# davidesantangelo/krep

Measured on AMD Instinct MI355X. Metric: GB/s scanned (literal scan, match offsets produced), haystack resident in HBM, higher is better.
Workload: dtype u8; 1 GPU; literal8: 8-byte case-sensitive literal 'Sherlock', ~1e-4 matches/byte, offsets tracked; 32 GiB per GPU (BASELINE.json configs[1]); pattern=Sherlock, bytes_per_gpu=34359738368, matches=3436005, parallelism=contiguous shards x1, start-offset ownership, 1 RCCL all-reduce of counts

## Files before the change

### include/krep_gpu_debug.h

```cpp
#ifndef KREP_GPU_DEBUG_H
#define KREP_GPU_DEBUG_H
#include "krep_gpu.h"
#ifdef __cplusplus
extern "C" {
#endif

uint64_t krep_gpu_debug_replay_host(int krep_ref_algo, const void *text, size_t n, const void *pattern, uint32_t m,
                                    int whole_word, size_t cur, int open_line);
void krep_gpu_debug_force_rounds(int rounds);
void krep_gpu_debug_force_stage_cap(int records);
void krep_gpu_debug_force_single_grid(int blocks);
uint64_t krep_gpu_debug_single_failovers(void);
uint64_t krep_gpu_debug_single_launches(void);
uint64_t krep_gpu_debug_tiny_launches(void);
uint64_t krep_gpu_debug_tiny_dense_launches(void);
void krep_gpu_debug_inject_failure(int kind);
void krep_gpu_debug_chain_fixups(uint64_t *rescans, uint64_t *replays);
void krep_gpu_debug_fold_carry(const krep_gpu_seq_carry_t *in, const krep_gpu_seq_carry_t *piece, krep_gpu_seq_carry_t *out);
uint64_t krep_gpu_debug_anchored_launches(void);
uint64_t krep_gpu_debug_literal_dma_launches(void);
int krep_gpu_debug_literal_dma_state(const krep_gpu_plan_t *plan, int *looked, int *barred, double *pass_rate);
uint64_t krep_gpu_debug_runs_launches(void);
int krep_gpu_debug_split_state(const krep_gpu_plan_t *plan);
int krep_gpu_debug_anchor_info(const krep_gpu_plan_t *plan, int *state, uint32_t *moved, double *rate_end_grams, double *rate_anchors);
int krep_gpu_debug_anchor_measured(const krep_gpu_plan_t *plan, double *measured, int *resamples);

#ifdef __cplusplus
}
#endif
#endif
```

### krep_amd/csrc/kg_config.hip

```cpp
#include <hip/hip_runtime.h>

#include <algorithm>
#include <atomic>
#include <chrono>
#include <cstdarg>
#include <cstdio>
#include <cstdlib>
#include <cstring>
#include <mutex>
#include <string>
#include <vector>

#include "../../include/krep_gpu.h"
#include "kg_common.h"
#include "kg_internal.h"
#include "kg_plan.h"
#include "kg_replay.h"

using namespace kg;

static thread_local std::string g_err;
namespace kg {
int fail(const char *fmt, ...)
{
// ... 204 lines not shown
namespace kg {
extern int g_s1_force_grid;
std::atomic<uint64_t> g_fused1_failovers{0};
}
extern "C" void krep_gpu_debug_force_single_grid(int blocks) { kg::g_s1_force_grid = blocks < 0 ? 0 : blocks; }
extern "C" uint64_t krep_gpu_debug_single_failovers(void) { return g_fused1_failovers.load(); }
namespace kg {
std::atomic<uint64_t> g_fused1_launches{0};
}
extern "C" uint64_t krep_gpu_debug_single_launches(void) { return kg::g_fused1_launches.load(); }
namespace kg {
std::atomic<uint64_t> g_tiny_launches{0};
}
extern "C" uint64_t krep_gpu_debug_tiny_launches(void) { return kg::g_tiny_launches.load(); }
namespace kg {
std::atomic<uint64_t> g_tiny_dense_launches{0};
}
extern "C" uint64_t krep_gpu_debug_tiny_dense_launches(void) { return kg::g_tiny_dense_launches.load(); }
namespace kg {
std::atomic<uint64_t> g_ac_anchored_launches{0};
}
extern "C" uint64_t krep_gpu_debug_anchored_launches(void) { return kg::g_ac_anchored_launches.load(); }
extern "C" uint64_t krep_gpu_debug_literal_dma_launches(void) { return kg::g_lit_dma_launches.load(); }
extern "C" uint64_t krep_gpu_debug_runs_launches(void) { return kg::g_runs_launches.load(); }
```

### krep_amd/csrc/kg_internal.h

```cpp
#pragma once
#include <hip/hip_runtime.h>

#include <atomic>
#include <cstring>
#include <initializer_list>
#include <mutex>
#include <vector>

#include "../../include/krep_gpu.h"
#include "../../include/krep_gpu_debug.h"
#include "kg_common.h"

namespace kg {

int fail(const char *fmt, ...);
const char *device_unusable(int device);
bool inject(int kind);
#define HIPCHK(x)                                                                                 \
    do                                                                                            \
    {                                                                                             \
        hipError_t e_ = (x);                                                                      \
        if (e_ != hipSuccess)                                                                     \
            return kg::fail("%s failed: %s (%s:%d)", #x, hipGetErrorString(e_), __FILE__, __LINE__); \
    } while (0)
// ... 24 lines not shown

template <auto Kernel> hipError_t grant_dynamic_lds(int bytes)
{
    static std::atomic<bool> granted[64];
    int dev = 0;
    (void)hipGetDevice(&dev);
    const bool known = dev >= 0 && dev < 64;
    if (known && granted[dev].load(std::memory_order_acquire))
        return hipSuccess;
    const hipError_t e = hipFuncSetAttribute(reinterpret_cast<const void *>(Kernel), hipFuncAttributeMaxDynamicSharedMemorySize, bytes);
    if (e == hipSuccess && known)
        granted[dev].store(true, std::memory_order_release);
    return e;
}

hipError_t launch_literal(const LitArgs &a, uint32_t num_cu, hipStream_t st);
int runs_count_greedy(const uint8_t *d_text, uint64_t text_len, uint64_t lo, uint64_t hi, uint32_t m, uint8_t byte, bool ci, int num_cu,
                      unsigned long long *d_slots, unsigned long long *h_slots, hipStream_t st, uint64_t *total, uint64_t *end_p1);
bool literal_dma_eligible(const LitArgs &a);
hipError_t launch_literal_dma(const LitArgs &a, uint32_t num_cu, hipStream_t st);
hipError_t launch_dma_byte_look(const uint8_t *text, uint64_t lo, uint32_t n_cells, uint32_t prefilter, bool ci, unsigned long long *out, hipStream_t st);
extern std::atomic<uint64_t> g_runs_launches;
extern std::atomic<uint64_t> g_lit_dma_launches;

struct PostScratch;
constexpr int kFusedShapeMax = 5;
double single_fused_max_density(int shape);
int single_fused_shape_for(double density, double margin, int start);
bool single_fused_reopens(uint64_t total, uint64_t span);
constexpr int kFusedGaveUp = 1;
int single_fused_run(const LitArgs &a, uint64_t n_units, uint64_t span, PostScratch &post, Counters *d_ctr, Counters *h_ctr,
                     uint32_t num_cu, int *shape, hipEvent_t ev_end, hipStream_t st, bool count_launch);

struct PostScratch
{
    unsigned long long *d_unitinfo = nullptr;
    unsigned long long *d_offsets = nullptr;
    unsigned long long *d_blk = nullptr;
    uint64_t units_cap = 0;
    unsigned long long *d_stage = nullptr;
    uint64_t stage_cap_words = 0;
    uint64_t *d_occ = nullptr;
    uint64_t occ_cap = 0;
    uint8_t *d_keep = nullptr;
    unsigned long long *d_gblk = nullptr;
    unsigned long long *d_surv = nullptr;
// ... 119 lines not shown
```

### krep_amd/csrc/kg_literal_dma.hip

```cpp
#include <hip/hip_runtime.h>
#include <algorithm>
#include <atomic>
#include <cstdlib>
#include "kg_common.h"
#include "kg_device.h"
#include "kg_internal.h"

namespace kg {

namespace {

constexpr u32 kDmaPark = 80;
constexpr u32 kDmaRing = 2u * kSegBytes;
constexpr u32 kDmaTail = 256u;
constexpr u32 kDmaWaveLds = kDmaRing + kDmaTail;
}

template <int KIND, bool MASKED, bool CI>
__global__ __launch_bounds__(kBlock, 2) void lit_scan_dma(const LitArgs a)
{
    extern __shared__ __attribute__((aligned(16))) uint8_t d_smem[];
    __shared__ u64 s_info_all[kWavesPerBlk][kDmaPark];
    __shared__ __attribute__((aligned(16))) unsigned short s_slots_all[kWavesPerBlk][kDmaPark * 16u];
    __shared__ u32 s_unit_all[kWavesPerBlk][kDmaPark];
    const u32 lane = lane_id();
    const u32 wave = __builtin_amdgcn_readfirstlane(threadIdx.x >> 6);
    uint8_t *ring = d_smem + wave * kDmaWaveLds;
    uint8_t *tailb = ring + kDmaRing;
    u64 *s_info = s_info_all[wave];
    unsigned short *s_slots = s_slots_all[wave];
    u32 *s_unit = s_unit_all[wave];
    const u32 ring_lds = (u32)(size_t)(__attribute__((address_space(3))) uint8_t *)ring;

    const bool want_pos = (a.flags & F_POS) != 0;
    const bool ww = (a.flags & F_WW) != 0;
    const u64 hi_match = (a.own_hi < a.text_len - a.m + 1) ? a.own_hi : (a.text_len - a.m + 1);
    constexpr u64 kUnitBytes = (u64)kRoundsBig * kSegBytes;
    const u64 n_units = a.num_tiles * kWavesPerBlk;

    const bool park = want_pos && a.stage_cap >= 16u && a.stage_cap <= 128u && (a.stage_cap & 7u) == 0u && n_units < (1ull << 32);
    const u32 park_max = park ? kDmaPark * 16u / a.stage_cap : 0u;
    u32 n_park = 0;
    auto flush_parked = [&]() __attribute__((always_inline)) {
        for (u32 i = lane; i < n_park; i += 64u)
        {
            const u64 u = s_unit[i];
            a.unitinfo[u] = s_info[i];
            if (s_info[i] & kUiCountMask)
            {
// ... 17 lines not shown
        const u64 u = static_next;
        static_next += (u64)gridDim.x * kWavesPerBlk;
        return u;
    };
    auto issue_round = [&](u64 seg, u32 buf) -> bool {
        if (seg + kSegBytes > a.text_len)
            return false;
        const uint8_t *src = a.text + seg + lane * 16u;
        uint8_t *dst = ring + buf * kSegBytes;
#pragma unroll
        for (int j = 0; j < kCells; ++j)
            __builtin_amdgcn_global_load_lds((const __attribute__((address_space(1))) void *)(src + j * kCellBytes),
                                             (__attribute__((address_space(3))) void *)(dst + j * kCellBytes), 16, 0, 2 );
        return true;
    };
    auto issue_tail = [&](u64 at) -> bool {
        if (at + kDmaTail > a.text_len)
            return false;
        __builtin_amdgcn_global_load_lds((const __attribute__((address_space(1))) void *)(a.text + at + lane * 4u),
                                         (__attribute__((address_space(3))) void *)tailb, 4, 0, 0);
        return true;
    };

    u64 acc_total = 0;
    u32 pf_cells = 0;
    u32 wcnt = 0;
    auto stage_hit = [&](u64 unit, u32 idx, u32 rel) __attribute__((always_inline)) {
        if (idx < a.stage_cap)
        {
            unsigned short *slot = park ? &s_slots[n_park * a.stage_cap] : reinterpret_cast<unsigned short *>(a.stage) + unit * (u64)a.stage_cap;
            slot[idx] = (unsigned short)rel;
        }
    };
    auto publish = [&](u64 unit) __attribute__((always_inline)) {
        acc_total += wcnt;
        if (want_pos)
        {
            if (lane == 0)
            {
                const u64 info = (u64)wcnt | (wcnt ? (kLnHead | kLnTail) : 0ull);
                if (park)
                {
                    s_info[n_park] = info;
                    s_unit[n_park] = (u32)unit;
                }
                else
                    a.unitinfo[unit] = info;
                if (wcnt > a.stage_cap)
                {
                    atomicAdd(&a.ctr->overflow_units, 1ull);
                    atomicMax(&a.ctr->max_unit_count, (u64)wcnt);
                }
            }
            if (park && ++n_park == park_max)
                flush_parked();
        }
        wcnt = 0;
    };
    auto exact = [&](u32 A0, u32 A4) -> bool {
        const u32 e0 = CI ? (A0 | a.l0) : A0;
        bool h = (KIND == 4 && MASKED) ? (((e0 ^ a.p0) & a.k0) == 0u) : (e0 == a.p0);
        if (KIND >= 8)
        {
            const u32 e4 = CI ? (A4 | a.l1) : A4;
            h = h && ((KIND == 8 && MASKED) ? (((e4 ^ a.p1) & a.k1) == 0u) : (e4 == a.p1));
        }
        return h;
    };
    auto owned = [&](u64 p) -> bool { return p >= a.own_lo && p < hi_match && !(p >= a.excl_lo && p < a.excl_hi); };
    auto word_ok = [&](u64 p) -> bool {
        if (p > 0 && p != a.ww_exempt_left && is_wordc(a.text[p - 1]))
            return false;
        if (p + a.m < a.text_len && is_wordc(a.text[p + a.m]))
            return false;
        return true;
    };
    auto boundary = [&](u64 seg_prev, u64 unit, u32 r_prev, u32 c0, u32 c1, u32 n0, u32 n1) __attribute__((always_inline)) {
        {
            const u32 f = 0x01010101u * ((CI ? (a.p0 | 0x20u) : a.p0) & 0xffu);
            const u32 y0 = (CI ? (c0 | 0x20202020u) : c0) ^ f, y1 = (CI ? (c1 | 0x20202020u) : c1) ^ f;
// ... 75 lines not shown
                             : "+v"(x[0]), "+v"(x[1]), "+v"(x[2]), "+v"(x[3]), "+v"(x[4]), "+v"(x[5]), "+v"(x[6]), "+v"(x[7]), "+v"(y[0]), "+v"(y[1]),
                               "+v"(y[2]), "+v"(y[3]), "+v"(y[4]), "+v"(y[5]), "+v"(y[6]), "+v"(y[7])
                             :
                             : "memory");
#pragma unroll
                for (int j = 0; j < kCells; ++j)
                {
                    vv[j] = make_uint4(x[j].x, x[j].y, x[j].z, x[j].w);
                    nn[j] = make_uint2(y[j].x, y[j].y);
                }
            }
            else
            {
#pragma unroll
                for (int j = 0; j < kCells; ++j)
                {
                    const W6 w = load_window_guarded(a.text, a.text_len, seg + (u64)j * kCellBytes + (u64)lane * 16u);
                    vv[j] = make_uint4(w.v[0], w.v[1], w.v[2], w.v[3]);
                    nn[j] = make_uint2(w.v[4], w.v[5]);
                }
            }
            if (deferred)
            {
                boundary(seg - kSegBytes, u0 + ((g - 1u) >> 2), (g - 1u) & 3u, c0, c1, __builtin_amdgcn_readfirstlane(vv[0].x),
                         __builtin_amdgcn_readfirstlane(vv[0].y));
                deferred = false;
                if (r == 0u)
                    publish(unit - 1u);
            }
            __builtin_amdgcn_sched_barrier(0);
#pragma unroll
            for (int j = 0; j < kCells; ++j)
            {
                const u64 lbase = seg + (u64)j * kCellBytes + (u64)lane * 16u;
                const u32 D[6] = {vv[j].x, vv[j].y, vv[j].z, vv[j].w, nn[j].x, nn[j].y};
                auto A = [&](int k) -> u32 {
                    return ((k & 3) == 0) ? D[k >> 2] : __builtin_amdgcn_alignbyte(D[(k >> 2) + 1], D[k >> 2], (u32)(k & 3));
                };
                u32 Dq[6];
#pragma unroll
                for (int w = 0; w < 6; ++w)
                    Dq[w] = CI ? (D[w] | 0x20202020u) : D[w];
                auto Aq = [&](int k) -> u32 {
                    return ((k & 3) == 0) ? Dq[k >> 2] : __builtin_amdgcn_alignbyte(Dq[(k >> 2) + 1], Dq[k >> 2], (u32)(k & 3));
                };
                const u32 p0q = CI ? (a.p0 | 0x20202020u) : a.p0;
                if (a.prefilter)
// ... 60 lines not shown
                            m16 &= ~(1u << k);
                    }
                }
                if (!__ballot(m16 != 0u))
                    continue;
                const u32 cnt = __popc(m16);
                u32 idx = wcnt, tot = 0;
                auto plane = [&](int b) {
                    const u64 bm = __ballot((cnt >> b) & 1u);
                    idx += mbcnt64(bm) << b;
                    tot += (u32)__popcll(bm) << b;
                };
                plane(0);
                plane(1);
                if (__ballot(cnt > 3u))
                {
                    plane(2);
                    plane(3);
                    plane(4);
                }
                wcnt += tot;
                if (want_pos)
                {
                    const u32 rel0 = (r * (u32)kCells + (u32)j) * kCellBytes + lane * 16u;
                    u32 rest = m16;
                    while (rest)
                    {
                        const u32 k = __builtin_ctz(rest);
                        rest &= rest - 1u;
                        stage_hit(unit, idx++, rel0 + k);
                    }
                }
            }
            if (dma_cur)
            {
                c0 = __builtin_amdgcn_readlane(vv[kCells - 1].z, 63);
                c1 = __builtin_amdgcn_readlane(vv[kCells - 1].w, 63);
                deferred = true;
            }
            if (g + 1u == nr)
            {
                if (deferred)
                {
                    u32 n0 = 0, n1 = 0;
                    if (tail_ok)
                    {
                        typedef u32 v2 __attribute__((ext_vector_type(2)));
                        v2 t;
                        const u32 taddr = ring_lds + kDmaRing;
                        asm volatile("ds_read_b64 %0, %1\n\ts_waitcnt lgkmcnt(0)" : "=v"(t) : "v"(taddr) : "memory");
                        n0 = __builtin_amdgcn_readfirstlane(t.x);
                        n1 = __builtin_amdgcn_readfirstlane(t.y);
                    }
                    else
                    {
                        const W6 w = load_window_guarded(a.text, a.text_len, seg + kSegBytes);
                        n0 = __builtin_amdgcn_readfirstlane(w.v[0]);
                        n1 = __builtin_amdgcn_readfirstlane(w.v[1]);
                    }
                    boundary(seg, unit, r, c0, c1, n0, n1);
                    deferred = false;
                }
                publish(unit);
            }
            else if (!deferred && r == 3u)
                publish(unit);
            dma_cur = dma_nx;
        }
        u0 = u_next;
    }
    if (park && n_park)
        flush_parked();
    if (lane == 0 && acc_total)
        atomicAdd(&a.ctr->total, acc_total);
    if (lane == 0 && pf_cells)
        atomicAdd(&a.ctr->candidates, (u64)pf_cells);
}

__global__ __launch_bounds__(256) void dma_byte_look(const uint8_t *text, u64 lo, u32 n_cells, u32 b4, u32 fold, unsigned long long *out)
{
    const u32 lane = lane_id();
    const u32 wave = blockIdx.x * 4u + (threadIdx.x >> 6), n_waves = gridDim.x * 4u;
    u32 cnt = 0;
    for (u32 c = wave; c < n_cells; c += n_waves)
    {
        const uint4 v = *reinterpret_cast<const uint4 *>(text + lo + (u64)c * kCellBytes + lane * 16u);
        const u32 d[4] = {v.x, v.y, v.z, v.w};
        u32 z = 0;
#pragma unroll
        for (int w = 0; w < 4; ++w)
        {
            const u32 y = (d[w] | fold) ^ b4;
            z |= (y - 0x01010101u) & ~y;
        }
        if (__ballot((z & 0x80808080u) != 0u))
            ++cnt;
    }
    if (lane == 0 && cnt)
        atomicAdd(out, (u64)cnt);
}
hipError_t launch_dma_byte_look(const uint8_t *text, uint64_t lo, uint32_t n_cells, uint32_t prefilter, bool ci, unsigned long long *out, hipStream_t st)
{
    hipLaunchKernelGGL(dma_byte_look, dim3(256), dim3(256), 0, st, text, (u64)lo, n_cells, prefilter, ci ? 0x20202020u : 0u, out);
    return hipGetLastError();
}

std::atomic<uint64_t> g_lit_dma_launches{0};

template <int KIND, bool MASKED, bool CI>
static hipError_t dma_launch3(const LitArgs &a, u32 num_cu, hipStream_t st)
{
    constexpr u32 lds = kWavesPerBlk * kDmaWaveLds;
    if (const hipError_t e = grant_dynamic_lds<&lit_scan_dma<KIND, MASKED, CI>>((int)lds); e != hipSuccess)
        return e;
    static const u32 bpc = [] { const char *e = getenv("KREP_GPU_LIT_DMA_BLOCKS_PER_CU"); return e && atoi(e) > 0 ? (u32)atoi(e) : 2u; }();
    const u32 grid = (u32)std::min<u64>(a.num_tiles, (u64)num_cu * bpc);
    hipLaunchKernelGGL((lit_scan_dma<KIND, MASKED, CI>), dim3(grid ? grid : 1), dim3(kBlock), lds, st, a);
    g_lit_dma_launches.fetch_add(1, std::memory_order_relaxed);
    return hipGetLastError();
}
template <int KIND, bool MASKED>
static hipError_t dma_launch2(const LitArgs &a, u32 num_cu, hipStream_t st)
{
    return (a.flags & F_CI) ? dma_launch3<KIND, MASKED, true>(a, num_cu, st) : dma_launch3<KIND, MASKED, false>(a, num_cu, st);
}

bool literal_dma_eligible(const LitArgs &a)
{
    return !getenv("KREP_GPU_LIT_NO_DMA") && a.prefilter != 0u && a.m >= 2 && a.m <= 8 && a.rounds == (u32)kRoundsBig && !(a.flags & F_LINES) && !a.emit_mode &&
           (a.upt >= 4 || getenv("KREP_GPU_LIT_DMA_ALL")) && a.text_len >= 4u * kSegBytes;
}
hipError_t launch_literal_dma(const LitArgs &a, u32 num_cu, hipStream_t st)
{
    if (a.m < 4)
        return dma_launch2<4, true>(a, num_cu, st);
    if (a.m == 4)
        return dma_launch2<4, false>(a, num_cu, st);
    if (a.m < 8)
        return dma_launch2<8, true>(a, num_cu, st);
    return dma_launch2<8, false>(a, num_cu, st);
}

}
```

### krep_amd/csrc/kg_plan.h

```cpp
#pragma once
#include <hip/hip_runtime.h>

#include <vector>

#include "../../include/krep_gpu.h"
#include "kg_common.h"
#include "kg_internal.h"

struct krep_gpu_plan
{
    krep_gpu_config_t cfg{};
    int device = 0;
    int ref_algo = KREP_RA_NONE;
    const char *unsupported = nullptr;
    bool only_matching = false;
    bool cs = true, ww = false, lines = false, track = false;
    size_t max_count = SIZE_MAX;
    std::vector<std::vector<uint8_t>> pats;
    uint32_t m = 0, p0 = 0, p1 = 0, k0 = 0, k1 = 0, l0 = 0, l1 = 0;
    uint32_t p2 = 0, p3 = 0, k2 = 0, k3 = 0, l2 = 0, l3 = 0;
    std::vector<uint8_t> pat_folded;
    bool has_border = false;
    bool has_newline = false;
    uint8_t *d_pat = nullptr;
    unsigned long long *d_pat_chunks = nullptr;
    uint32_t n_chunks = 0;
    kg::Counters *d_ctr = nullptr, *h_ctr = nullptr;
    int num_cu = 256;
    hipEvent_t ev0 = nullptr, ev1 = nullptr;
    kg::AcTables *ac = nullptr;
    kg::AcTables *ac_long = nullptr, *ac_short = nullptr;
    int ac_split = 0;
    match_position_t *d_split_rec = nullptr;
    uint64_t split_cap = 0;
    bool ac_has_newline = false;
    kg::PostScratch post;
    uint32_t sparse_cap = 16;
    bool dma_look_done = false;
    bool dma_off = false;
    const void *dma_off_text = nullptr;
    size_t dma_off_len = 0;
    double dma_pass_rate = 0;
    bool first_look_done = false;
    bool fused1_ok = true;
    bool fusedk_on = false;
    bool fusedk_never = false;
    int fusedk_shape = 0;
    int fused1_shape = 0;
    match_position_t *d_nl_rec = nullptr;
    uint64_t *d_nl_ln = nullptr;
    uint64_t nl_cap = 0;
    bool lines_list_off = false;
    kg::PostScratch aux;
    search_params_t sp{};
    std::vector<const char *> pat_ptrs;
    std::vector<size_t> pat_lens;
};
namespace kg {
struct Window
{
    const uint8_t *d_text;
    size_t text_len;
    size_t own_lo, own_hi;
    size_t global_base;
    size_t global_len;
// ... 7 lines not shown
```

### krep_amd/csrc/kg_scan.hip

```cpp
#include <hip/hip_runtime.h>

#include <algorithm>
#include <cstdio>
#include <cstdlib>
#include <cstring>
#include <vector>

#include "../../include/krep_gpu.h"
#include "kg_common.h"
#include "kg_internal.h"
#include "kg_plan.h"
#include "kg_replay.h"

using namespace kg;

struct Verdict { uint64_t ret, store; };
static Verdict verdict_for(int algo, const krep_gpu_plan *pl, uint64_t total, uint64_t lines, bool have_result)
{
    const size_t maxc = pl->max_count;
    const bool store = pl->track && have_result;
    Verdict v{0, 0};
    switch (algo)
    {
    case KREP_RA_MEMCHR:
// ... 213 lines not shown
          ps.excl_lo == ps.excl_hi && L.span() >= (1ull << 30) && !getenv("KREP_GPU_NO_FIRST_LOOK")))
        return 0;
    pl->first_look_done = true;
    const uint64_t span = L.span(), win = 2ull << 20, tile_bytes = (uint64_t)kRoundsBig * kSegBytes * kWavesPerBlk;
    HIPCHK(hipMemsetAsync(pl->d_ctr, 0, sizeof(Counters), st));
    uint64_t looked = 0;
    for (int q = 0; q < 2; ++q)
    {
        LitArgs sm = a;
        sm.flags &= ~(uint32_t)(F_POS | F_LINES);
        sm.stage_cap = 0;
        sm.upt = 0;
        sm.emit_mode = 0;
        sm.own_lo = (a.anchor + span / 4 * (2 * q + 1)) & ~(uint64_t)15;
        sm.own_hi = std::min<uint64_t>(L.hi_match, sm.own_lo + win);
        sm.anchor = sm.own_lo;
        sm.num_tiles = (sm.own_hi - sm.anchor + tile_bytes - 1) / tile_bytes;
        looked += sm.own_hi - sm.own_lo;
        HIPCHK(launch_literal(sm, (uint32_t)pl->num_cu, st));
    }
    HIPCHK(hipMemcpyAsync(pl->h_ctr, pl->d_ctr, sizeof(Counters), hipMemcpyDeviceToHost, st));
    HIPCHK(hipStreamSynchronize(st));
    const double density = looked ? (double)pl->h_ctr->total / (double)looked : 0.0, per_unit = density * 32768.0;
    if (m_scan == 1)
    {
        if (density > single_fused_max_density(kFusedShapeMax))
            pl->fused1_ok = false;
        else
            pl->fused1_shape = single_fused_shape_for(density, 1.05, 0);
    }
    else if (m_scan <= 8 && !pl->fusedk_never && per_unit >= fusedk_min_hits_per_unit() &&
             density <= single_fused_max_density(kFusedShapeMax))
    {
        pl->fusedk_on = true;
        pl->fusedk_shape = single_fused_shape_for(density, 1.05, 0);
    }
    else if (per_unit > 6.0)
        pl->sparse_cap = std::max<uint32_t>(pl->sparse_cap, per_unit > 100.0 ? 256u : per_unit > 40.0 ? 128u : 64u);
    if (getenv("KREP_GPU_DEBUG"))
        fprintf(stderr, "krep-gpu: first look: %.2f hits per 32-KiB unit in %llu sampled bytes -> one-pass %d (shape %d / %d), staging slot %u\n", per_unit,
                (unsigned long long)looked, (int)(m_scan == 1 ? pl->fused1_ok : pl->fusedk_on), pl->fused1_shape, pl->fusedk_shape, pl->sparse_cap);
    if ((a.flags & F_POS) && !L.fsc)
        a.stage_cap = a.rounds == kRoundsBig ? (m_scan == 1 ? 512u : pl->sparse_cap) : a.stage_cap;
    return 0;
}

// ... 15 lines not shown
    if (rc == 2)
        return 2;
    if (rc != kFusedGaveUp)
    {
        res->total = pl->h_ctr->total;
        res->summary = res->total ? (kLnHead | kLnTail) : 0;
        if (m_scan != 1 && L.density(res->total) * 32768.0 < 0.5 * fusedk_min_hits_per_unit())
            pl->fusedk_on = false;
        *done = true;
        return 0;
    }
    if (m_scan == 1)
        pl->fused1_ok = false;
    else
        pl->fusedk_on = false, pl->fusedk_never = true;
    g_fused1_failovers.fetch_add(1);
    return 0;
}

static void lit_learn_density(krep_gpu_plan *pl, const LitPass &ps, const LitScan &L)
{
    const LitArgs &a = L.a;
    const uint32_t m_scan = a.m;
    if ((a.flags & F_POS) && m_scan != 1 && a.rounds == kRoundsBig && pl->h_ctr->overflow_units * 64 > L.n_units && !L.fsc)
    {
        uint32_t want = 64;
        if (pl->sparse_cap >= 64)
            for (want = 128; want < 256 && want < pl->h_ctr->max_unit_count; want *= 2) {}
        pl->sparse_cap = std::max(pl->sparse_cap, want);
    }
    if ((a.flags & F_POS) && m_scan >= 2 && m_scan <= 8 && a.rounds == kRoundsBig && !L.fsc && !pl->fusedk_never &&
        ps.sink == LitPass::RECORDS && !ps.lines && L.hi_match > a.anchor)
    {
        const double density = L.density(pl->h_ctr->total);
        if (density * 32768.0 >= fusedk_min_hits_per_unit() && density <= single_fused_max_density(kFusedShapeMax))
        {
            pl->fusedk_on = true;
            pl->fusedk_shape = single_fused_shape_for(density, 1.0, 0);
        }
    }
    if (getenv("KREP_GPU_DEBUG") && (a.flags & F_POS))
        fprintf(stderr, "krep-gpu: literal scan: %llu of %llu units overflowed a %u-entry slot (fullest: %llu); one-pass next: %d (shape %d)\n",
                pl->h_ctr->overflow_units, (unsigned long long)L.n_units, a.stage_cap, pl->h_ctr->max_unit_count, (int)pl->fusedk_on,
                pl->fusedk_shape);
}
static void lit_reopen(krep_gpu_plan *pl, const LitScan &L)
{
    const uint32_t m_scan = L.a.m;
    if (!pl->fused1_ok && m_scan == 1 && single_fused_reopens(pl->h_ctr->total, L.span()))
        pl->fused1_ok = true;
    if (pl->fusedk_never && m_scan >= 2 && m_scan <= 8 && single_fused_reopens(pl->h_ctr->total, L.span()))
        pl->fusedk_never = false;
}

static int lit_two_pass(krep_gpu_plan *pl, const Window &w, const LitPass &ps, LitScan &L, bool chain, hipStream_t st)
{
    LitArgs &a = L.a;
    a.positions = ps.d_out;
    a.pos_cap = ps.sink == LitPass::RECORDS ? ps.out_cap : 0;
    HIPCHK(launch_literal(a, (uint32_t)pl->num_cu, st));
    if (chain && post_order(*ps.post, L.n_units, a.stage_cap, a.m, a.anchor + w.global_base, L.unit_bytes(), ps.lines, ps.d_out, a.pos_cap,
                            pl->d_ctr, pl->num_cu, st))
        return 2;
    if (ps.ev_end) HIPCHK(hipEventRecord(ps.ev_end, st));
    HIPCHK(hipMemcpyAsync(pl->h_ctr, pl->d_ctr, sizeof(Counters), hipMemcpyDeviceToHost, st));
    HIPCHK(hipStreamSynchronize(st));
    lit_dma_rate(pl, w, L);
    lit_learn_density(pl, ps, L);
    if ((a.flags & F_POS) && pl->h_ctr->overflow_units)
    {
        LitArgs e = a;
        e.emit_mode = 1;
        HIPCHK(hipMemsetAsync(&pl->d_ctr->ticket, 0, sizeof(unsigned long long), st));
        HIPCHK(launch_literal(e, (uint32_t)pl->num_cu, st));
        if (ps.ev_end) HIPCHK(hipEventRecord(ps.ev_end, st));
// ... 26 lines not shown
        }
    }
    return 0;
}

static int lit_pass(krep_gpu_plan *pl, const Window &w, const LitPass &ps, hipStream_t st, LitResult *res)
{
    *res = LitResult{};
    const uint32_t m_scan = ps.first_byte ? 1u : pl->m;
    size_t own_hi = std::min(ps.own_hi, w.text_len);
    if (ps.first_byte)
        own_hi = std::min<size_t>(own_hi, w.text_len - pl->m + 1);
    const uint64_t hi_match = std::min<uint64_t>(own_hi, w.text_len - m_scan + 1);
    if (hi_match <= ps.own_lo)
        return 0;
    LitScan L = lit_args(pl, w, ps, own_hi, hi_match);
    if (lit_dma_look(pl, w, ps, L, st))
        return 2;
    res->n_units = L.n_units;
    res->unit_bytes = L.unit_bytes();
    res->anchor = L.a.anchor;
    bool done = false;
    if (lit_first_look(pl, ps, L, st) || lit_one_pass(pl, w, ps, L, st, res, &done))
        return 2;
    if (done)
        return 0;
    const bool chain = (L.a.flags & (F_POS | F_LINES)) != 0;
    if (chain)
    {
        PostScratch &post = *ps.post;
        if (post_reserve(post, L.n_units, (L.n_units * L.a.stage_cap + 3) / 4))
            return 2;
        L.a.unitinfo = post.d_unitinfo;
        L.a.stage = (uint64_t *)post.d_stage;
        L.a.offsets = (const uint64_t *)post.d_offsets;
    }
    HIPCHK(hipMemsetAsync(pl->d_ctr, 0, sizeof(Counters), st));
    if (ps.sink != LitPass::OCC ? lit_two_pass(pl, w, ps, L, chain, st) : lit_two_pass_occ(pl, w, ps, L, st))
        return 2;
    res->total = pl->h_ctr->total;
    res->lines = pl->h_ctr->lines;
    lit_reopen(pl, L);
    res->summary = chain ? pl->h_ctr->summary : (res->total ? (kLnHead | kLnTail) : 0);
    return 0;
}

// ... 774 lines not shown
```

### krep_amd/csrc/kg_tickets.h

```cpp
#pragma once
#include <hip/hip_runtime.h>
#include "kg_common.h"
#include "kg_device.h"

namespace kg {

constexpr unsigned long long kTkReady = 1ull << 63;
constexpr uint32_t kTkSpinLimit = 1u << 24;
constexpr uint32_t kTkResolveChunk = 8;

__device__ __forceinline__ void tk_resolve(unsigned long long *__restrict__ agg, unsigned long long *__restrict__ pref,
                                           const unsigned long long n_tickets, Counters *ctr, const uint32_t lane)
{
    u64 running = 0, base = 0;
    u32 spins = 0;
    while (base < n_tickets)
    {
        const u64 mine = base + (u64)lane * kTkResolveChunk;
        u64 v[kTkResolveChunk];
        u32 lead = 0, nvalid = 0;
        bool run = true;
#pragma unroll
        for (u32 k = 0; k < kTkResolveChunk; ++k)
        {
// ... 56 lines not shown
__device__ __forceinline__ unsigned long long tk_wait_prefix(const unsigned long long *__restrict__ pref, const unsigned long long t,
                                                              Counters *ctr, const uint32_t lane)
{
    u64 p = 0;
    if (lane == 0)
    {
        for (uint32_t spins = 0;; ++spins)
        {
            p = __hip_atomic_load(&pref[t], __ATOMIC_RELAXED, __HIP_MEMORY_SCOPE_AGENT);
            if (p & kTkReady)
                break;
            if (spins > 2u * kTkSpinLimit)
            {
                atomicAdd(&ctr->overflow_units, 1ull);
                p = kTkReady;
                break;
            }
            __builtin_amdgcn_s_sleep(4);
        }
    }
    return rfl64(p) & ~kTkReady;
}

}
```

### krep_amd/engine.py

```python
from __future__ import annotations

import ctypes as C
import os

import numpy as np

from . import abi

HERE = os.path.dirname(os.path.abspath(__file__))
LIB_PATH = os.path.join(HERE, "lib", "libkrep_gpu.so")


class KrepGpuError(RuntimeError):
    pass


class Engine:

    def __init__(self, path: str = LIB_PATH):
        path = os.environ.get("KREP_GPU_LIB", path)
        if not os.path.exists(path):
            raise KrepGpuError(f"{path} is missing: build it with `python -m krep_amd.build` "
                               "(hipcc --offload-arch=gfx950); there is no CPU fallback")
        if not os.environ.get("KREP_GPU_NO_TORCH"):
# ... 82 lines not shown
        L.krep_gpu_comm_init_rank.argtypes = [C.c_void_p, C.c_int, C.c_int, C.c_int]
        L.krep_gpu_comm_allreduce_u64.restype = C.c_int
        L.krep_gpu_comm_allreduce_u64.argtypes = [C.POINTER(C.c_uint64), C.c_int]
        L.krep_gpu_comm_allreduce_device_u64.restype = C.c_int
        L.krep_gpu_comm_allreduce_device_u64.argtypes = [C.c_void_p, C.c_int, C.c_void_p]
        L.krep_gpu_comm_destroy.restype = None
        L.krep_gpu_rccl_calls.restype = C.c_uint64
        L.krep_gpu_rccl_version.restype = C.c_int
        L.krep_gpu_debug_force_single_grid.restype = None
        L.krep_gpu_debug_force_single_grid.argtypes = [C.c_int]
        L.krep_gpu_debug_single_failovers.restype = C.c_uint64
        L.krep_gpu_debug_single_launches.restype = C.c_uint64
        L.krep_gpu_debug_tiny_launches.restype = C.c_uint64
        L.krep_gpu_debug_chain_fixups.restype = None
        L.krep_gpu_debug_chain_fixups.argtypes = [C.POINTER(C.c_uint64), C.POINTER(C.c_uint64)]
        L.krep_gpu_debug_tiny_dense_launches.restype = C.c_uint64
        if hasattr(L, "krep_gpu_debug_anchor_info"):
            L.krep_gpu_debug_anchored_launches.restype = C.c_uint64
            L.krep_gpu_debug_literal_dma_launches.restype = C.c_uint64
            L.krep_gpu_debug_runs_launches.restype = C.c_uint64
            L.krep_gpu_debug_anchor_info.restype = C.c_int
            L.krep_gpu_debug_anchor_info.argtypes = [C.c_void_p, C.POINTER(C.c_int), C.POINTER(C.c_uint32), C.POINTER(C.c_double),
                                                     C.POINTER(C.c_double)]
        if hasattr(L, "krep_gpu_alloc_placed"):
            L.krep_gpu_alloc_placed.restype = C.c_int
            L.krep_gpu_alloc_placed.argtypes = [C.c_int, C.c_size_t, C.c_size_t, C.c_int, C.POINTER(C.c_void_p), C.POINTER(C.c_void_p),
                                                C.POINTER(abi.Placement)]
            L.krep_gpu_free_placed.restype = C.c_int
            L.krep_gpu_free_placed.argtypes = [C.c_int, C.c_void_p]
        if hasattr(L, "krep_gpu_debug_literal_dma_state"):
            L.krep_gpu_debug_literal_dma_state.restype = C.c_int
            L.krep_gpu_debug_literal_dma_state.argtypes = [C.c_void_p, C.POINTER(C.c_int), C.POINTER(C.c_int), C.POINTER(C.c_double)]
        if hasattr(L, "krep_gpu_debug_anchor_measured"):
            L.krep_gpu_debug_anchor_measured.restype = C.c_int
            L.krep_gpu_debug_anchor_measured.argtypes = [C.c_void_p, C.POINTER(C.c_double), C.POINTER(C.c_int)]
        L.krep_gpu_last_shard_info.restype = None
        L.krep_gpu_last_shard_info.argtypes = [C.POINTER(abi.ShardInfo)]
        L.krep_gpu_available.restype = C.c_int
        L.krep_gpu_unavailable_reason.restype = C.c_char_p
        L.krep_gpu_last_status.restype = C.c_int
        L.krep_gpu_set_cpu_fallback.restype = None
        L.krep_gpu_set_cpu_fallback.argtypes = [C.c_void_p]
        L.krep_gpu_worthwhile.restype = C.c_int
        L.krep_gpu_worthwhile.argtypes = [C.POINTER(abi.SearchParams), C.c_size_t]
        L.krep_gpu_worthwhile_ex.restype = C.c_int
        L.krep_gpu_worthwhile_ex.argtypes = [C.POINTER(abi.SearchParams), C.c_size_t, C.c_int]
# ... 28 lines not shown
    def force_single_grid(self, blocks: int):
        self.lib.krep_gpu_debug_force_single_grid(blocks)

    def single_failovers(self) -> int:
        return int(self.lib.krep_gpu_debug_single_failovers())

    def single_launches(self) -> int:
        return int(self.lib.krep_gpu_debug_single_launches())

    def chain_fixups(self):
        a, b = C.c_uint64(0), C.c_uint64(0)
        self.lib.krep_gpu_debug_chain_fixups(C.byref(a), C.byref(b))
        return int(a.value), int(b.value)

    def tiny_dense_launches(self) -> int:
        return int(self.lib.krep_gpu_debug_tiny_dense_launches())

    def runs_launches(self) -> int:
        return int(self.lib.krep_gpu_debug_runs_launches())

    def literal_dma_launches(self) -> int:
        return int(self.lib.krep_gpu_debug_literal_dma_launches())

    def alloc_placed(self, text_bytes: int, record_bytes: int, tries: int = 3, device: int = 0):
        t, r, info = C.c_void_p(0), C.c_void_p(0), abi.Placement()
        if self.lib.krep_gpu_alloc_placed(device, text_bytes, record_bytes, tries, C.byref(t), C.byref(r), C.byref(info)):
            raise KrepGpuError("krep_gpu_alloc_placed failed: " + self.last_error())
        return int(t.value), int(r.value or 0), info

    def free_placed(self, d_text: int, device: int = 0):
        if self.lib.krep_gpu_free_placed(device, C.c_void_p(d_text)):
            raise KrepGpuError("krep_gpu_free_placed failed: " + self.last_error())

    def anchored_launches(self) -> int:
        return int(self.lib.krep_gpu_debug_anchored_launches())

    def tiny_launches(self) -> int:
        return int(self.lib.krep_gpu_debug_tiny_launches())

    def force_stage_cap(self, c: int):
        self.lib.krep_gpu_debug_force_stage_cap(c)

    def default_config(self) -> abi.Config:
        c = abi.Config()
        self.lib.krep_gpu_config_default(C.byref(c))
        return c
# ... 300 lines not shown
```

Measured before the change: 6570 GB/s.

## Add one-pass DMA literal scan with decoupled-lookback ticket prefixes

```diff
diff --git a/include/krep_gpu_debug.h b/include/krep_gpu_debug.h
--- a/include/krep_gpu_debug.h
+++ b/include/krep_gpu_debug.h
@@ -19,6 +19,9 @@
 void krep_gpu_debug_fold_carry(const krep_gpu_seq_carry_t *in, const krep_gpu_seq_carry_t *piece, krep_gpu_seq_carry_t *out);
 uint64_t krep_gpu_debug_anchored_launches(void);
 uint64_t krep_gpu_debug_literal_dma_launches(void);
+uint64_t krep_gpu_debug_literal_dma_one_pass_launches(void);
+uint64_t krep_gpu_debug_literal_dma_one_pass_failovers(void);
+void krep_gpu_debug_force_literal_dma_grid(int blocks);
 int krep_gpu_debug_literal_dma_state(const krep_gpu_plan_t *plan, int *looked, int *barred, double *pass_rate);
 uint64_t krep_gpu_debug_runs_launches(void);
 int krep_gpu_debug_split_state(const krep_gpu_plan_t *plan);
diff --git a/krep_amd/csrc/kg_config.hip b/krep_amd/csrc/kg_config.hip
--- a/krep_amd/csrc/kg_config.hip
+++ b/krep_amd/csrc/kg_config.hip
@@ -250,4 +250,7 @@
 }
 extern "C" uint64_t krep_gpu_debug_anchored_launches(void) { return kg::g_ac_anchored_launches.load(); }
 extern "C" uint64_t krep_gpu_debug_literal_dma_launches(void) { return kg::g_lit_dma_launches.load(); }
+extern "C" uint64_t krep_gpu_debug_literal_dma_one_pass_launches(void) { return kg::g_lit_dma1p_launches.load(); }
+extern "C" uint64_t krep_gpu_debug_literal_dma_one_pass_failovers(void) { return kg::g_lit_dma1p_failovers.load(); }
+extern "C" void krep_gpu_debug_force_literal_dma_grid(int blocks) { kg::g_lit_dma1p_force_grid = blocks < 0 ? 0 : blocks; }
 extern "C" uint64_t krep_gpu_debug_runs_launches(void) { return kg::g_runs_launches.load(); }
diff --git a/krep_amd/csrc/kg_internal.h b/krep_amd/csrc/kg_internal.h
--- a/krep_amd/csrc/kg_internal.h
+++ b/krep_amd/csrc/kg_internal.h
@@ -70,6 +70,12 @@
 hipError_t launch_dma_byte_look(const uint8_t *text, uint64_t lo, uint32_t n_cells, uint32_t prefilter, bool ci, unsigned long long *out, hipStream_t st);
 extern std::atomic<uint64_t> g_runs_launches;
 extern std::atomic<uint64_t> g_lit_dma_launches;
+hipError_t launch_literal_dma_one_pass(const LitArgs &a, unsigned long long *d_agg, unsigned long long *d_pref, uint64_t n_tickets,
+                                       uint32_t num_cu, hipStream_t st);
+uint32_t lit_dma_one_pass_list();
+extern std::atomic<uint64_t> g_lit_dma1p_launches;
+extern std::atomic<uint64_t> g_lit_dma1p_failovers;
+extern int g_lit_dma1p_force_grid;
 
 struct PostScratch;
 constexpr int kFusedShapeMax = 5;
diff --git a/krep_amd/csrc/kg_literal_dma.hip b/krep_amd/csrc/kg_literal_dma.hip
--- a/krep_amd/csrc/kg_literal_dma.hip
+++ b/krep_amd/csrc/kg_literal_dma.hip
@@ -5,6 +5,7 @@
 #include "kg_common.h"
 #include "kg_device.h"
 #include "kg_internal.h"
+#include "kg_tickets.h"
 
 namespace kg {
 
@@ -14,17 +15,37 @@
 constexpr u32 kDmaRing = 2u * kSegBytes;
 constexpr u32 kDmaTail = 256u;
 constexpr u32 kDmaWaveLds = kDmaRing + kDmaTail;
-}
-
-template <int KIND, bool MASKED, bool CI>
-__global__ __launch_bounds__(kBlock, 2) void lit_scan_dma(const LitArgs a)
+constexpr u32 kOpHits = 768;
+constexpr u32 kOpTk = 32;
+static_assert(kOpHits * 4u + kOpTk * 12u <= kDmaPark * 44u, "the one-pass mode's static LDS stays within the staging mode's (two workgroups per CU)");
+static_assert(kOpTk <= 64u, "one lane per parked ticket picks its prefix up");
+}
+uint32_t lit_dma_one_pass_list() { return kOpHits; }
+
+template <int KIND, bool MASKED, bool CI, bool ONEP>
+__global__ __launch_bounds__(kBlock, 2) void lit_scan_dma(const LitArgs a, u64 *__restrict__ agg, const u64 *__restrict__ pref, const u64 n_tickets)
 {
     extern __shared__ __attribute__((aligned(16))) uint8_t d_smem[];
-    __shared__ u64 s_info_all[kWavesPerBlk][kDmaPark];
-    __shared__ __attribute__((aligned(16))) unsigned short s_slots_all[kWavesPerBlk][kDmaPark * 16u];
-    __shared__ u32 s_unit_all[kWavesPerBlk][kDmaPark];
+    __shared__ u64 s_info_all[kWavesPerBlk][ONEP ? 1u : kDmaPark];
+    __shared__ __attribute__((aligned(16))) unsigned short s_slots_all[kWavesPerBlk][ONEP ? 8u : kDmaPark * 16u];
+    __shared__ u32 s_unit_all[kWavesPerBlk][ONEP ? 1u : kDmaPark];
+    __shared__ u32 s_hits_all[kWavesPerBlk][ONEP ? kOpHits : 1u];
+    __shared__ u32 s_tk_all[kWavesPerBlk][ONEP ? 3u * kOpTk : 1u];
     const u32 lane = lane_id();
     const u32 wave = __builtin_amdgcn_readfirstlane(threadIdx.x >> 6);
+    if (ONEP && wave == 0)
+    {
+        u64 r = 1;
+        if (lane == 0)
+            r = __hip_atomic_fetch_add(&a.ctr->pad[0], 1ull, __ATOMIC_RELAXED, __HIP_MEMORY_SCOPE_AGENT);
+        if (rfl64(r) == 0ull)
+        {
+            tk_resolve(agg, const_cast<u64 *>(pref), n_tickets, a.ctr, lane);
+            return;
+        }
+    }
+    u32 *s_hits = s_hits_all[wave];
+    u32 *s_tk = s_tk_all[wave];
     uint8_t *ring = d_smem + wave * kDmaWaveLds;
     uint8_t *tailb = ring + kDmaRing;
     u64 *s_info = s_info_all[wave];
@@ -88,17 +109,69 @@
         return true;
     };
 
+    u32 hp = 0;
+    u32 used = 0;
+    u32 n_tkp = 0;
+    bool overflowed = false;
+    auto hwrap = [](const u32 x) -> u32 { return x >= kOpHits ? x - kOpHits : x; };
+    auto flush_records = [&](const u32 n_out) __attribute__((always_inline)) {
+        u64 pfx = 0;
+        if (lane < n_out)
+            pfx = tk_wait_prefix_lane(pref, (u64)s_tk[3u * lane], a.ctr);
+        for (u32 i = 0; i < n_out; ++i)
+        {
+            const u32 t = __builtin_amdgcn_readfirstlane(s_tk[3u * i]), cnt = __builtin_amdgcn_readfirstlane(s_tk[3u * i + 1u]),
+                      at = __builtin_amdgcn_readfirstlane(s_tk[3u * i + 2u]);
+            const u64 first = ((u64)(u32)__builtin_amdgcn_readlane((u32)(pfx >> 32), i) << 32) | (u32)__builtin_amdgcn_readlane((u32)pfx, i);
+            const u64 tbase = a.global_base + a.anchor + (u64)t * ((u64)tk_units * kUnitBytes);
+            const u32 pad = (u32)(first & 7ull);
+            for (u32 q = lane; q < cnt + pad; q += 64u)
+            {
+                if (q < pad)
+                    continue;
+                const u32 e = q - pad;
+                const u64 idx = first + e;
+                if (idx < a.pos_cap)
+                {
+                    const u64 st = tbase + s_hits[hwrap(at + e)], en = st + a.m;
+                    typedef u32 u32x4 __attribute__((ext_vector_type(4)));
+                    const u32x4 rec = {(u32)st, (u32)(st >> 32), (u32)en, (u32)(en >> 32)};
+                    __builtin_nontemporal_store(rec, reinterpret_cast<u32x4 *>(a.positions + 2 * idx));
+                }
+            }
+            used -= cnt;
+        }
+        if (n_out < n_tkp)
+        {
+            const u32 t = s_tk[3u * n_out], cnt = s_tk[3u * n_out + 1u], at = s_tk[3u * n_out + 2u];
+            if (lane == 0)
+            {
+                s_tk[0] = t;
+                s_tk[1] = cnt;
+                s_tk[2] = at;
+            }
+        }
+        n_tkp -= n_out;
+    };
+
     u64 acc_total = 0;
     u32 pf_cells = 0;
     u32 wcnt = 0;
     auto stage_hit = [&](u64 unit, u32 idx, u32 rel) __attribute__((always_inline)) {
-        if (idx < a.stage_cap)
+        if (ONEP)
+        {
+            if (idx < kOpHits - used)
+                s_hits[hwrap(hp + idx)] = rel;
+        }
+        else if (idx < a.stage_cap)
         {
             unsigned short *slot = park ? &s_slots[n_park * a.stage_cap] : reinterpret_cast<unsigned short *>(a.stage) + unit * (u64)a.stage_cap;
             slot[idx] = (unsigned short)rel;
         }
     };
     auto publish = [&](u64 unit) __attribute__((always_inline)) {
+        if (ONEP)
+            return;
         acc_total += wcnt;
         if (want_pos)
         {
@@ -122,6 +195,29 @@
                 flush_parked();
         }
         wcnt = 0;
+    };
+    auto end_ticket = [&](u32 t) __attribute__((always_inline)) {
+        if (lane == 0)
+            __hip_atomic_store(&agg[t], (u64)wcnt | kTkReady, __ATOMIC_RELAXED, __HIP_MEMORY_SCOPE_AGENT);
+        u32 fresh = 0;
+        if (wcnt > kOpHits - used)
+            overflowed = true;
+        else if (wcnt)
+        {
+            if (lane == 0)
+            {
+                s_tk[3u * n_tkp] = t;
+                s_tk[3u * n_tkp + 1u] = wcnt;
+                s_tk[3u * n_tkp + 2u] = hp;
+            }
+            ++n_tkp;
+            hp = hwrap(hp + wcnt);
+            used += wcnt;
+            fresh = 1;
+        }
+        wcnt = 0;
+        if ((n_tkp == kOpTk || used > kOpHits / 2u) && n_tkp > fresh)
+            flush_records(n_tkp - fresh);
     };
     auto exact = [&](u32 A0, u32 A4) -> bool {
         const u32 e0 = CI ? (A0 | a.l0) : A0;
@@ -243,7 +339,7 @@
             }
             if (deferred)
             {
-                boundary(seg - kSegBytes, u0 + ((g - 1u) >> 2), (g - 1u) & 3u, c0, c1, __builtin_amdgcn_readfirstlane(vv[0].x),
+                boundary(seg - kSegBytes, u0 + ((g - 1u) >> 2), ONEP ? g - 1u : (g - 1u) & 3u, c0, c1, __builtin_amdgcn_readfirstlane(vv[0].x),
                          __builtin_amdgcn_readfirstlane(vv[0].y));
                 deferred = false;
                 if (r == 0u)
@@ -350,7 +446,7 @@
                 wcnt += tot;
                 if (want_pos)
                 {
-                    const u32 rel0 = (r * (u32)kCells + (u32)j) * kCellBytes + lane * 16u;
+                    const u32 rel0 = ((ONEP ? g : r) * (u32)kCells + (u32)j) * kCellBytes + lane * 16u;
                     u32 rest = m16;
                     while (rest)
                     {
@@ -386,10 +482,13 @@
                         n0 = __builtin_amdgcn_readfirstlane(w.v[0]);
                         n1 = __builtin_amdgcn_readfirstlane(w.v[1]);
                     }
-                    boundary(seg, unit, r, c0, c1, n0, n1);
+                    boundary(seg, unit, ONEP ? g : r, c0, c1, n0, n1);
                     deferred = false;
                 }
-                publish(unit);
+                if (ONEP)
+                    end_ticket((u32)u0 / tk_units);
+                else
+                    publish(unit);
             }
             else if (!deferred && r == 3u)
                 publish(unit);
@@ -397,8 +496,12 @@
         }
         u0 = u_next;
     }
-    if (park && n_park)
+    if (!ONEP && park && n_park)
         flush_parked();
+    if (ONEP && n_tkp)
+        flush_records(n_tkp);
+    if (ONEP && overflowed && lane == 0)
+        atomicAdd(&a.ctr->overflow_units, 1ull);
     if (lane == 0 && acc_total)
         atomicAdd(&a.ctr->total, acc_total);
     if (lane == 0 && pf_cells)
@@ -434,23 +537,42 @@
 }
 
 std::atomic<uint64_t> g_lit_dma_launches{0};
-
-template <int KIND, bool MASKED, bool CI>
-static hipError_t dma_launch3(const LitArgs &a, u32 num_cu, hipStream_t st)
+std::atomic<uint64_t> g_lit_dma1p_launches{0};
+std::atomic<uint64_t> g_lit_dma1p_failovers{0};
+int g_lit_dma1p_force_grid = 0;
+
+template <int KIND, bool MASKED, bool CI, bool ONEP>
+static hipError_t dma_launch4(const LitArgs &a, u64 *agg, const u64 *pref, u64 n_tickets, u32 num_cu, hipStream_t st)
 {
     constexpr u32 lds = kWavesPerBlk * kDmaWaveLds;
-    if (const hipError_t e = grant_dynamic_lds<&lit_scan_dma<KIND, MASKED, CI>>((int)lds); e != hipSuccess)
+    if (const hipError_t e = grant_dynamic_lds<&lit_scan_dma<KIND, MASKED, CI, ONEP>>((int)lds); e != hipSuccess)
         return e;
     static const u32 bpc = [] { const char *e = getenv("KREP_GPU_LIT_DMA_BLOCKS_PER_CU"); return e && atoi(e) > 0 ? (u32)atoi(e) : 2u; }();
-    const u32 grid = (u32)std::min<u64>(a.num_tiles, (u64)num_cu * bpc);
-    hipLaunchKernelGGL((lit_scan_dma<KIND, MASKED, CI>), dim3(grid ? grid : 1), dim3(kBlock), lds, st, a);
+    u32 grid = (u32)std::min<u64>(a.num_tiles, (u64)num_cu * bpc);
+    if (ONEP && g_lit_dma1p_force_grid > 0)
+        grid = std::min<u32>(grid, (u32)g_lit_dma1p_force_grid);
+    hipLaunchKernelGGL((lit_scan_dma<KIND, MASKED, CI, ONEP>), dim3(grid ? grid : 1), dim3(kBlock), lds, st, a, agg, pref, n_tickets);
     g_lit_dma_launches.fetch_add(1, std::memory_order_relaxed);
+    if (ONEP)
+        g_lit_dma1p_launches.fetch_add(1, std::memory_order_relaxed);
     return hipGetLastError();
 }
-template <int KIND, bool MASKED>
-static hipError_t dma_launch2(const LitArgs &a, u32 num_cu, hipStream_t st)
-{
-    return (a.flags & F_CI) ? dma_launch3<KIND, MASKED, true>(a, num_cu, st) : dma_launch3<KIND, MASKED, false>(a, num_cu, st);
+template <int KIND, bool MASKED, bool ONEP>
+static hipError_t dma_launch2(const LitArgs &a, u64 *agg, const u64 *pref, u64 n_tickets, u32 num_cu, hipStream_t st)
+{
+    return (a.flags & F_CI) ? dma_launch4<KIND, MASKED, true, ONEP>(a, agg, pref, n_tickets, num_cu, st)
+                            : dma_launch4<KIND, MASKED, false, ONEP>(a, agg, pref, n_tickets, num_cu, st);
+}
+template <bool ONEP>
+static hipError_t dma_launch1(const LitArgs &a, u64 *agg, const u64 *pref, u64 n_tickets, u32 num_cu, hipStream_t st)
+{
+    if (a.m < 4)
+        return dma_launch2<4, true, ONEP>(a, agg, pref, n_tickets, num_cu, st);
+    if (a.m == 4)
+        return dma_launch2<4, false, ONEP>(a, agg, pref, n_tickets, num_cu, st);
+    if (a.m < 8)
+        return dma_launch2<8, true, ONEP>(a, agg, pref, n_tickets, num_cu, st);
+    return dma_launch2<8, false, ONEP>(a, agg, pref, n_tickets, num_cu, st);
 }
 
 bool literal_dma_eligible(const LitArgs &a)
@@ -460,13 +582,15 @@
 }
 hipError_t launch_literal_dma(const LitArgs &a, u32 num_cu, hipStream_t st)
 {
-    if (a.m < 4)
-        return dma_launch2<4, true>(a, num_cu, st);
-    if (a.m == 4)
-        return dma_launch2<4, false>(a, num_cu, st);
-    if (a.m < 8)
-        return dma_launch2<8, true>(a, num_cu, st);
-    return dma_launch2<8, false>(a, num_cu, st);
-}
-
-}
+    return dma_launch1<false>(a, nullptr, nullptr, 0, num_cu, st);
+}
+hipError_t launch_literal_dma_one_pass(const LitArgs &a, unsigned long long *d_agg, unsigned long long *d_pref, uint64_t n_tickets, u32 num_cu,
+                                       hipStream_t st)
+{
+    const u64 n_units = a.num_tiles * kWavesPerBlk;
+    if (!(a.flags & F_POS) || !a.upt || n_units >= (1ull << 32) || n_tickets != (n_units + a.upt - 1) / a.upt || (u64)a.upt * kRoundsBig * kSegBytes > (1ull << 31))
+        return hipErrorInvalidValue;
+    return dma_launch1<true>(a, d_agg, d_pref, n_tickets, num_cu, st);
+}
+
+}
diff --git a/krep_amd/csrc/kg_plan.h b/krep_amd/csrc/kg_plan.h
--- a/krep_amd/csrc/kg_plan.h
+++ b/krep_amd/csrc/kg_plan.h
@@ -41,6 +41,10 @@
     const void *dma_off_text = nullptr;
     size_t dma_off_len = 0;
     double dma_pass_rate = 0;
+    bool dma1p_off = false;
+    const void *dma1p_off_text = nullptr;
+    size_t dma1p_off_len = 0;
+    double lit_density = -1.0;
     bool first_look_done = false;
     bool fused1_ok = true;
     bool fusedk_on = false;
diff --git a/krep_amd/csrc/kg_scan.hip b/krep_amd/csrc/kg_scan.hip
--- a/krep_amd/csrc/kg_scan.hip
+++ b/krep_amd/csrc/kg_scan.hip
@@ -259,6 +259,7 @@
     HIPCHK(hipMemcpyAsync(pl->h_ctr, pl->d_ctr, sizeof(Counters), hipMemcpyDeviceToHost, st));
     HIPCHK(hipStreamSynchronize(st));
     const double density = looked ? (double)pl->h_ctr->total / (double)looked : 0.0, per_unit = density * 32768.0;
+    pl->lit_density = density;
     if (m_scan == 1)
     {
         if (density > single_fused_max_density(kFusedShapeMax))
@@ -320,6 +321,8 @@
 {
     const LitArgs &a = L.a;
     const uint32_t m_scan = a.m;
+    if (L.span() >= 8 * L.unit_bytes() && !ps.first_byte)
+        pl->lit_density = L.density(pl->h_ctr->total);
     if ((a.flags & F_POS) && m_scan != 1 && a.rounds == kRoundsBig && pl->h_ctr->overflow_units * 64 > L.n_units && !L.fsc)
     {
         uint32_t want = 64;
@@ -349,6 +352,59 @@
         pl->fused1_ok = true;
     if (pl->fusedk_never && m_scan >= 2 && m_scan <= 8 && single_fused_reopens(pl->h_ctr->total, L.span()))
         pl->fusedk_never = false;
+}
+
+static int lit_dma_one_pass(krep_gpu_plan *pl, const Window &w, const LitPass &ps, LitScan &L, hipStream_t st, LitResult *res, bool *done)
+{
+    *done = false;
+    if (!(ps.sink == LitPass::RECORDS && !ps.lines && !ps.first_byte && ps.excl_lo == ps.excl_hi && L.fsc == 0 && !getenv("KREP_GPU_LIT_DMA_TWO_PASS")))
+        return 0;
+    LitArgs a = L.a;
+    if (!a.upt && getenv("KREP_GPU_LIT_DMA_ALL") && !getenv("KREP_GPU_LIT_UPT"))
+        a.upt = 8;
+    if (!a.upt || !literal_dma_eligible(a) || L.n_units >= (1ull << 32))
+        return 0;
+    if (pl->dma1p_off && pl->dma1p_off_text == (const void *)w.d_text && pl->dma1p_off_len == w.text_len)
+        return 0;
+    const uint64_t ticket_bytes = (uint64_t)a.upt * L.unit_bytes();
+    const double gate = std::min(0.25 * (double)lit_dma_one_pass_list(), fusedk_min_hits_per_unit() * (double)a.upt);
+    if (pl->lit_density >= 0.0 && pl->lit_density * (double)ticket_bytes >= gate)
+        return 0;
+    constexpr uint64_t kCtrWords = 16;
+    static_assert(sizeof(Counters) <= kCtrWords * sizeof(unsigned long long), "the counters in front of the ticket arrays");
+    const uint64_t n_tk = (L.n_units + a.upt - 1) / a.upt, cap_tk = n_tk + kCtrWords / 2;
+    PostScratch &post = *ps.post;
+    HIPCHK(grow_scratch(post.tk_cap, cap_tk, cap_tk, {dev_buf(post.d_tk, 2 * cap_tk * sizeof(unsigned long long))}));
+    Counters *d_ctr = reinterpret_cast<Counters *>(post.d_tk);
+    unsigned long long *d_agg = post.d_tk + kCtrWords, *d_pref = d_agg + n_tk;
+    a.ctr = d_ctr;
+    a.positions = ps.d_out;
+    a.pos_cap = ps.out_cap;
+    a.stage_cap = 0;
+    HIPCHK(hipMemsetAsync(post.d_tk, 0, (kCtrWords + 2 * n_tk) * sizeof(unsigned long long), st));
+    HIPCHK(launch_literal_dma_one_pass(a, d_agg, d_pref, n_tk, (uint32_t)pl->num_cu, st));
+    if (ps.ev_end) HIPCHK(hipEventRecord(ps.ev_end, st));
+    HIPCHK(hipMemcpyAsync(pl->h_ctr, d_ctr, sizeof(Counters), hipMemcpyDeviceToHost, st));
+    HIPCHK(hipStreamSynchronize(st));
+    LitScan La = L;
+    La.a = a;
+    lit_dma_rate(pl, w, La);
+    if (pl->h_ctr->overflow_units)
+    {
+        pl->dma1p_off = true;
+        pl->dma1p_off_text = w.d_text;
+        pl->dma1p_off_len = w.text_len;
+        g_lit_dma1p_failovers.fetch_add(1);
+        if (getenv("KREP_GPU_DEBUG"))
+            fprintf(stderr, "krep-gpu: literal scan: a ticket overflowed the one-pass hit list -> the two-pass road for this text\n");
+        return 0;
+    }
+    if (L.span() >= ticket_bytes)
+        pl->lit_density = L.density(pl->h_ctr->total);
+    res->total = pl->h_ctr->total;
+    res->summary = res->total ? (kLnHead | kLnTail) : 0;
+    *done = true;
+    return 0;
 }
 
 static int lit_two_pass(krep_gpu_plan *pl, const Window &w, const LitPass &ps, LitScan &L, bool chain, hipStream_t st)
@@ -421,6 +477,10 @@
     res->anchor = L.a.anchor;
     bool done = false;
     if (lit_first_look(pl, ps, L, st) || lit_one_pass(pl, w, ps, L, st, res, &done))
+        return 2;
+    if (done)
+        return 0;
+    if (lit_dma_one_pass(pl, w, ps, L, st, res, &done))
         return 2;
     if (done)
         return 0;
diff --git a/krep_amd/csrc/kg_tickets.h b/krep_amd/csrc/kg_tickets.h
--- a/krep_amd/csrc/kg_tickets.h
+++ b/krep_amd/csrc/kg_tickets.h
@@ -102,4 +102,24 @@
     return rfl64(p) & ~kTkReady;
 }
 
+__device__ __forceinline__ unsigned long long tk_wait_prefix_lane(const unsigned long long *__restrict__ pref, const unsigned long long t,
+                                                                   Counters *ctr)
+{
+    u64 p = 0;
+    for (uint32_t spins = 0;; ++spins)
+    {
+        p = __hip_atomic_load(&pref[t], __ATOMIC_RELAXED, __HIP_MEMORY_SCOPE_AGENT);
+        if (p & kTkReady)
+            break;
+        if (spins > 2u * kTkSpinLimit)
+        {
+            atomicAdd(&ctr->overflow_units, 1ull);
+            p = kTkReady;
+            break;
+        }
+        __builtin_amdgcn_s_sleep(4);
+    }
+    return p & ~kTkReady;
 }
+
+}
diff --git a/krep_amd/engine.py b/krep_amd/engine.py
--- a/krep_amd/engine.py
+++ b/krep_amd/engine.py
@@ -128,6 +128,11 @@
             L.krep_gpu_debug_anchor_info.restype = C.c_int
             L.krep_gpu_debug_anchor_info.argtypes = [C.c_void_p, C.POINTER(C.c_int), C.POINTER(C.c_uint32), C.POINTER(C.c_double),
                                                      C.POINTER(C.c_double)]
+        if hasattr(L, "krep_gpu_debug_literal_dma_one_pass_launches"):
+            L.krep_gpu_debug_literal_dma_one_pass_launches.restype = C.c_uint64
+            L.krep_gpu_debug_literal_dma_one_pass_failovers.restype = C.c_uint64
+            L.krep_gpu_debug_force_literal_dma_grid.restype = None
+            L.krep_gpu_debug_force_literal_dma_grid.argtypes = [C.c_int]
         if hasattr(L, "krep_gpu_alloc_placed"):
             L.krep_gpu_alloc_placed.restype = C.c_int
             L.krep_gpu_alloc_placed.argtypes = [C.c_int, C.c_size_t, C.c_size_t, C.c_int, C.POINTER(C.c_void_p), C.POINTER(C.c_void_p),
@@ -202,6 +207,15 @@
     def literal_dma_launches(self) -> int:
         return int(self.lib.krep_gpu_debug_literal_dma_launches())
 
+    def literal_dma_one_pass_launches(self) -> int:
+        return int(self.lib.krep_gpu_debug_literal_dma_one_pass_launches())
+
+    def literal_dma_one_pass_failovers(self) -> int:
+        return int(self.lib.krep_gpu_debug_literal_dma_one_pass_failovers())
+
+    def force_literal_dma_grid(self, blocks: int):
+        self.lib.krep_gpu_debug_force_literal_dma_grid(blocks)
+
     def alloc_placed(self, text_bytes: int, record_bytes: int, tries: int = 3, device: int = 0):
         t, r, info = C.c_void_p(0), C.c_void_p(0), abi.Placement()
         if self.lib.krep_gpu_alloc_placed(device, text_bytes, record_bytes, tries, C.byref(t), C.byref(r), C.byref(info)):
```

After: 6687 GB/s (median of 6 runs). 1.02x the previous value.
